# VulcanClimateModeling/fv3net

Hardware: AMD Instinct MI355X
Metric: columns/s ML-tendency inference at C384x79 (Zhao-Carr dense emulator) (higher is better)
Workload: dtype f32

## Files before the change

fv3net_amd/csrc/mlp.hip:

```cpp
#include <cmath>
#include <cstddef>
#include <cstdlib>
#include <cstring>
#include <algorithm>
#include <type_traits>
#include <cfloat>
#include <vector>

#include "common.h"

namespace fv3hip {
namespace {

#define MLP_CHUNK_BARRIER() asm volatile("s_waitcnt lgkmcnt(0)\n\ts_barrier" ::: "memory")

#define MLP_SLOT_SCHED(NT, Q)                                                          \
    __builtin_amdgcn_sched_group_barrier(0x008, 1, 0);                                 \
    __builtin_amdgcn_sched_group_barrier(0x002 | 0x400, 64, 0);                        \
    _Pragma("unroll") for (int _i = 1; _i < (NT); ++_i)                                \
    {                                                                                  \
        __builtin_amdgcn_sched_group_barrier(0x008, 1, 0);                             \
        __builtin_amdgcn_sched_group_barrier(0x004 | 0x010 | 0x080, (Q), 0);           \
    }                                                                                  \
    __builtin_amdgcn_sched_barrier(0)

typedef float f32x16 __attribute__((ext_vector_type(16)));
typedef float f32x4 __attribute__((ext_vector_type(4)));

constexpr int kMaxSources = 16;
constexpr int kMaxOutputs = 32;
constexpr int kMaxK = 2048;
constexpr int kThreads = 256;
constexpr int kTileSamples = 128;

struct KEntry {
    int src;
    int feat;
    float center;
    float scale;
    int transform;
    float eps;
    int pad0, pad1;
};

struct XAddr {
    int64_t row;
    unsigned int ss;
    unsigned int pad;
};

struct XNorm {
    float center, rscale, eps;
    int flags;
};

struct OFast {
    int64_t row;
    float scale, center;
};
struct OSlow {
    float lo, hi, mask;
    unsigned int ss;
};
struct ORes {
    int64_t src_row;
    int64_t out_row;
    unsigned int src_ss, out_ss, pad0, pad1;
};

struct OEntry {
    float scale, center, lo, hi;
    float mask;
    int out_feat;
    int res;
    int pad0;
};

struct MlpLaunch {
    unsigned int w_bytes;
    const f32x4 *w;
    const KEntry *ktab;
    const OEntry *otab;
    const float *bias;
    int n_chunks1;
    int n_hidden;
    int n_otiles;
    int n_hout_tiles;
    int smallf_off;
    int smallf_n;
    int64_t sink;
    int n_ktab;
    int n_otab;
    int n_bias;
    int out64;
    int n_log_chunks;
    int n_logfast_chunks;
    int epi_fast;
    int has_limits;
    int n_residual;
    int64_t n_samples;
    int64_t n_tiles;
    unsigned long long *stamps;
    const void *src[kMaxSources];
    int64_t src_fs[kMaxSources];
    int64_t src_ss[kMaxSources];
    void *out[kMaxOutputs];
    int64_t out_fs[kMaxOutputs];
    int64_t out_ss[kMaxOutputs];
};

__host__ __device__ constexpr int rho(int r) { return (r & 3) + 8 * (r >> 2); }

#ifndef MLP_STAMP_PHASE
#define MLP_STAMP_PHASE 0
#endif
#ifdef MLP_STAMPS
#define SLOT_STAMP(phase, s)                                          \
    if ((phase) == MLP_STAMP_PHASE) {                                 \
        const unsigned long long t_ = __builtin_readcyclecounter();   \
        if ((s) > 0) sl_acc[(s) - 1] += t_ - sl_t;                    \
        sl_t = t_;                                                    \
    }
#define CHUNK_STAMP_END(phase, KC)                                    \
    if ((phase) == MLP_STAMP_PHASE) {                                 \
        const unsigned long long t_ = __builtin_readcyclecounter();   \
        sl_acc[(KC) - 1] += t_ - sl_t;                                \
        sl_acc[16] += 1;                                              \
    }
#else
#define SLOT_STAMP(phase, s) ((void)0)
#define CHUNK_STAMP_END(phase, KC) ((void)0)
#endif
template <int HT, bool SRC64, bool XBULK, bool HOUT, bool SMALLF, bool L1SHORT>
__global__ __launch_bounds__(kThreads, 1) void mlp_fused_kernel(const MlpLaunch p)
{
    constexpr int HG = (HT + 3) / 4;
    constexpr int KC_H = 16;
    constexpr int GS = (HT == 1) ? 4 : 8;
    constexpr int NGO = GS / 4;
    constexpr int KC_O = HT * 16 / GS;
    constexpr int CH_H = KC_H * HG * 64;
    constexpr int CH_O = KC_O * NGO * 64;
    constexpr int NV_H = CH_H / kThreads;
    constexpr int NV_O = CH_O / kThreads;
    constexpr int NV_MAX = (NV_H > NV_O) ? NV_H : NV_O;
    constexpr int CH_MAX = (CH_H > CH_O) ? CH_H : CH_O;
    constexpr bool EPI_SIDE = XBULK && KC_O >= 12;

    extern __shared__ __attribute__((aligned(16))) char smem[];
    f32x4 *wbuf = reinterpret_cast<f32x4 *>(smem);
    float *xs = reinterpret_cast<float *>(wbuf + 2 * CH_MAX);
    XAddr *xa_tab = reinterpret_cast<XAddr *>(xs + (XBULK ? 2 * 32 * kTileSamples : 0));
    XNorm *xn_tab = reinterpret_cast<XNorm *>(xa_tab + p.n_ktab);
    OFast *ofast = reinterpret_cast<OFast *>(xn_tab + p.n_ktab);
    OSlow *oslow = reinterpret_cast<OSlow *>(ofast + p.n_otab);
    ORes *ores = reinterpret_cast<ORes *>(oslow + p.n_otab);
    float *biasl = reinterpret_cast<float *>(ores + (p.n_residual ? p.n_otab : 0));

    const int tid = threadIdx.x;
    const int lane = tid & 63;
    const int wave = tid >> 6;
    const int half = lane >> 5;

    {
        typedef const int64_t __attribute__((address_space(4))) *KargPtr64;
        typedef const char __attribute__((address_space(4))) *KargBytes64;
        KargPtr64 ksrc = (KargPtr64)((KargBytes64)__builtin_amdgcn_kernarg_segment_ptr() + offsetof(MlpLaunch, src));
        for (int i = tid; i < p.n_ktab; i += kThreads) {
            const KEntry e = p.ktab[i];
            const int sidx = e.src < 0 ? 0 : e.src;
            const int64_t esz = SRC64 ? 8 : 4;
            XAddr a;
            a.row = e.src < 0 ? reinterpret_cast<int64_t>(p.bias)
                              : ksrc[sidx] + (int64_t)e.feat * ksrc[kMaxSources + sidx] * esz;
            a.ss = e.src < 0 ? 0u : (unsigned int)(ksrc[2 * kMaxSources + sidx] * esz);
            a.pad = 0;
            xa_tab[i] = a;
            XNorm nrm;
            nrm.center = e.src < 0 ? 0.f : e.center;
// ... 207 lines not shown
    };
    auto bulk_finish1 = [&](int c, int i, int buf, auto with_log) {
        bulk_finish_e(xn_tab[c * 32 + fr + 8 * i], i, buf, with_log);
    };
    int xb = 0;

    int64_t tile = blockIdx.x;
    if (tile >= p.n_tiles) return;

    {
        int64_t n = tile * kTileSamples + wave * 32 + (lane & 31);
        if (XBULK) bulk_issue(0, tile * kTileSamples); else issue_x(0, n < p.n_samples ? n : p.n_samples - 1);
#pragma unroll
        for (int part = 0; part < 2; ++part) {
            issue_w(0, part);
#pragma unroll
            for (int i = 0; i < NVH; ++i) commit_w1(0, part, i);
        }
        if (XBULK) {
            if (p.n_logfast_chunks > 0) {
#pragma unroll
                for (int i = 0; i < 4; ++i) bulk_finish1(0, i, 0, std::integral_constant<int, 2>{});
            } else {
#pragma unroll
                for (int i = 0; i < 4; ++i) bulk_finish1(0, i, 0, std::integral_constant<int, 1>{});
            }
        } else {
            finish_x(0);
        }
        __syncthreads();
#pragma unroll
        for (int j = 0; j < AG; ++j) a_cur[j] = wbuf[lane + j * 64];
    }
    float b_cur = XBULK ? xs[half * kTileSamples + wave * 32 + (lane & 31)] : 0.f;

    for (; tile < p.n_tiles; tile += gridDim.x) {
        const int64_t n = tile * kTileSamples + wave * 32 + (lane & 31);
        const bool valid = n < p.n_samples;
        const int64_t nc = valid ? n : p.n_samples - 1;
        const int64_t next_tile = tile + gridDim.x;
        int64_t nn = next_tile * kTileSamples + wave * 32 + (lane & 31);
        if (nn >= p.n_samples) nn = p.n_samples - 1;
        int g = 0;

        f32x16 h[HT];
        STAMP_BEGIN();
        {
#pragma unroll
            for (int t = 0; t < HT; ++t)
#pragma unroll
                for (int r = 0; r < 16; ++r) h[t][r] = biasl[(t * 16 + r) * 2 + half];
            using T_ = std::true_type;
            using F_ = std::false_type;
            const int L = p.n_log_chunks, NC = p.n_chunks1;
            using HT_c = std::integral_constant<int, HT>;
            using HG_c = std::integral_constant<int, HG>;
            using Q5_c = std::integral_constant<int, 5>;
            auto l1_chunk = [&](int c, int cn, auto with_log) __attribute__((always_inline)) {
                const int gnext = (g + 1 < G) ? g + 1 : 0;
                const XAddr *xa_n = xa_tab + 2 * cn * KC_H + half;
                const XNorm *xn_c = xn_tab + 2 * c * KC_H + half;
                const XNorm *xn_n = xn_tab + 2 * cn * KC_H + half;
                XAddr xa_cur = xa_n[0], xa_nxt = xa_cur;
                XNorm xn_cur = xn_c[2 * (KC_H / 2)], xn_nxt = xn_cur;
#pragma unroll
                for (int s = 0; s < KC_H; ++s) {
                    run_slot(h, HT_c{}, HG_c{}, Q5_c{}, s, KC_H, xcur[s], [&](int s_) {
                        if (s_ + 1 < KC_H) {
                            xa_nxt = xa_n[2 * (s_ + 1)];
                            xn_nxt = (s_ + 1 < KC_H / 2) ? xn_c[2 * (s_ + 1 + KC_H / 2)] : xn_n[2 * (s_ + 1 - KC_H / 2)];
                        }
                        issue_x1(xa_cur, s_, nc);
                        const int el = (s_ < KC_H / 2) ? s_ + KC_H / 2 : s_ - KC_H / 2;
                        if (decltype(with_log)::value) finish_x1(xn_cur, el); else finish_x1_plain(xn_cur, el);
                        stage_step(s_, KC_H, gnext, par ^ 1);
                        xa_cur = xa_nxt;
                        xn_cur = xn_nxt;
                    });
                }
                par ^= 1;
                ++g;
            };
            auto l1_chunk_bulk = [&](int cn, int64_t n0, auto with_log, auto kc1_c) __attribute__((always_inline)) {
                constexpr int KC1 = decltype(kc1_c)::value, FIN0 = (KC1 == 16) ? 8 : 3;
                const int gnext = (g + 1 < G) ? g + 1 : 0;
                const float *xsb = xs + xb * 32 * kTileSamples + half * kTileSamples + wave * 32 + (lane & 31);
                const float *xsn = xs + (xb ^ 1) * 32 * kTileSamples + half * kTileSamples + wave * 32 + (lane & 31);
                const unsigned int nb = bulk_sample(n0);
                XAddr xa4[4];
                XNorm xn4[4];
                typedef const XAddr __attribute__((address_space(3))) *LXAddr;
                typedef const XNorm __attribute__((address_space(3))) *LXNorm;
                LXAddr xa_c = (LXAddr)(xa_tab + cn * 32 + fr);
                LXNorm xn_c = (LXNorm)(xn_tab + cn * 32 + fr);
                asm volatile("" : "+v"(xa_c), "+v"(xn_c));
                const XAddr *xa_g = (const XAddr *)xa_c;
                const XNorm *xn_g = (const XNorm *)xn_c;
#pragma unroll
                for (int s = 0; s < KC1; ++s) {
                    SLOT_STAMP((int)decltype(with_log)::value, s);
                    run_slot(h, HT_c{}, HG_c{}, Q5_c{}, s, KC1, b_cur, [&](int s_) {
                        b_cur = (s_ + 1 < KC1) ? xsb[2 * (s_ + 1) * kTileSamples] : xsn[0];
                        if (s_ == 0) {
#pragma unroll
                            for (int i = 0; i < 4; ++i) xa4[i] = xa_g[8 * i];
                        }
                        if (s_ == 1) {
#pragma unroll
                            for (int i = 0; i < 4; ++i) bulk_issue1(xa4[i], i, nb);
                        }
                        if (s_ == FIN0) {
#pragma unroll
                            for (int i = 0; i < 4; ++i) xn4[i] = xn_g[8 * i];
                        }
                        if (s_ > FIN0 && s_ <= FIN0 + 4) bulk_finish_e(xn4[s_ - FIN0 - 1], s_ - FIN0 - 1, xb ^ 1, with_log);
                        stage_step(s_, KC1, gnext, par ^ 1);
                    });
                }
                CHUNK_STAMP_END((int)decltype(with_log)::value, KC1);
                par ^= 1;
                xb ^= 1;
                ++g;
            };
            if (XBULK) {
                const int64_t n0 = tile * kTileSamples;
                using M0_ = std::integral_constant<int, 0>;
                using M1_ = std::integral_constant<int, 1>;
                using M2_ = std::integral_constant<int, 2>;
                const int NF = p.n_logfast_chunks;
                using KC16_ = std::integral_constant<int, 16>;
                const int64_t n1 = (next_tile < p.n_tiles ? next_tile : tile) * kTileSamples;
                if constexpr (L1SHORT) {
                    l1_chunk_bulk(0, n1, M0_{}, std::integral_constant<int, 8>{});
                } else {
                    int c = 0;
                    for (; c + 1 < NF; ++c) l1_chunk_bulk(c + 1, n0, M2_{}, KC16_{});
                    for (; c + 1 < L; ++c) l1_chunk_bulk(c + 1, n0, M1_{}, KC16_{});
                    for (; c < NC - 1; ++c) l1_chunk_bulk(c + 1, n0, M0_{}, KC16_{});
                    if (NF > 0) l1_chunk_bulk(0, n1, M2_{}, KC16_{});
                    else if (L > 0) l1_chunk_bulk(0, n1, M1_{}, KC16_{});
                    else l1_chunk_bulk(0, n1, M0_{}, KC16_{});
                }
            } else {
                int c = 0;
                for (; c < L && c < NC - 1; ++c) l1_chunk(c, c + 1, T_{});
                for (; c < NC - 1; ++c) l1_chunk(c, c + 1, F_{});
                if (L > 0) l1_chunk(NC - 1, NC - 1, T_{}); else l1_chunk(NC - 1, NC - 1, F_{});
            }
#pragma unroll
            for (int t = 0; t < HT; ++t)
#pragma unroll
                for (int r = 0; r < 16; ++r) h[t][r] = (h[t][r] < 0.f) ? 0.f : h[t][r];
        }
        STAMP_END(0);
        for (int l = 1; l < p.n_hidden; ++l) {
            f32x16 h2[HT];
            const float *bl = biasl + l * HT * 32;
#pragma unroll
            for (int t = 0; t < HT; ++t)
#pragma unroll
                for (int r = 0; r < 16; ++r) h2[t][r] = bl[(t * 16 + r) * 2 + half];
#pragma unroll
            for (int kt = 0; kt < HT; ++kt) {
                const int gnext = (g + 1 < G) ? g + 1 : 0;
#pragma unroll
                for (int s = 0; s < KC_H; ++s) {
                    SLOT_STAMP(10, s);
                    run_slot(h2, std::integral_constant<int, HT>{}, std::integral_constant<int, HG>{},
                             std::integral_constant<int, 2>{}, s, KC_H, h[kt][s],
                             [&](int s_) { stage_step(s_, KC_H, gnext, par ^ 1); });
                }
                CHUNK_STAMP_END(10, KC_H);
                par ^= 1;
                ++g;
            }
#pragma unroll
            for (int t = 0; t < HT; ++t)
#pragma unroll
                for (int r = 0; r < 16; ++r) h[t][r] = (h2[t][r] < 0.f) ? 0.f : h2[t][r];
        }
        STAMP_END(1);
        {
            typedef f32x4 __attribute__((address_space(1))) *GF32x4;
            typedef const f32x4 __attribute__((address_space(1))) *GCF32x4;
            typedef d64x2 __attribute__((address_space(1))) *GF64x2;
            typedef const d64x2 __attribute__((address_space(1))) *GCF64x2;
            const int64_t n0t = tile * kTileSamples + wave * 32;
            const int e_wrow = lane >> 3, e_wcol = (lane & 7) * 4;
            constexpr int NHO = HOUT ? HT : 0;
            float *scr = xs + (xb ^ 1) * 32 * kTileSamples + wave * 1024;
            auto epi_put_tile = [&](const f32x16 &y) {
#pragma unroll
                for (int r = 0; r < 16; ++r) scr[(rho(r) + 4 * half) * 32 + (lane & 31)] = y[r];
            };
            auto epi_put4 = [&](int64_t row_addr, const f32x4 v) {
                if (p.out64) {
                    const d64x2 lo = {(double)v[0], (double)v[1]}, hi = {(double)v[2], (double)v[3]};
                    *(GF64x2)(row_addr + (n0t + e_wcol) * 8) = lo;
                    *(GF64x2)(row_addr + (n0t + e_wcol) * 8 + 16) = hi;
                } else {
                    *(GF32x4)(row_addr + (n0t + e_wcol) * 4) = v;
                }
            };
            auto epi_row = [&](const OFast of, f32x4 v, int idx, auto mode_c) {
                if (decltype(mode_c)::value != 0) {
                    *(GF32x4)(of.row + (n0t + e_wcol) * 4) = v;
                    return;
                }
                if (p.has_limits) {
                    const OSlow os = oslow[idx];
#pragma unroll
                    for (int q = 0; q < 4; ++q) {
                        float x = v[q];
                        if (x < os.lo) x = os.lo;
                        if (x >= os.hi) x = os.hi;
                        v[q] = x * os.mask;
                    }
                }
                if (of.row != 0) epi_put4(of.row, v);
                if (p.n_residual) {
                    const ORes e = ores[idx];
                    if (e.src_row != 0) {
                        f32x4 before;
                        if (SRC64) {
                            const d64x2 lo = *(GCF64x2)(e.src_row + (n0t + e_wcol) * 8);
                            const d64x2 hi = *(GCF64x2)(e.src_row + (n0t + e_wcol) * 8 + 16);
                            before[0] = (float)lo[0]; before[1] = (float)lo[1];
                            before[2] = (float)hi[0]; before[3] = (float)hi[1];
                        } else {
                            before = *(GCF32x4)(e.src_row + (n0t + e_wcol) * 4);
                        }
                        epi_put4(e.out_row, before + v);
                    }
                }
            };
            auto epi_fast_now = [&](const f32x16 &y, int t) {
                if (n0t >= p.n_samples) return;
                epi_put_tile(y);
#pragma unroll
                for (int j = 0; j < 4; ++j) {
                    const int row = e_wrow + 8 * j, idx = t * 32 + row;
                    epi_row(ofast[idx], *reinterpret_cast<const f32x4 *>(scr + row * 32 + e_wcol), idx, std::integral_constant<int, 0>{});
                }
            };
            OFast e_of[2];
            f32x4 e_v[2];
            constexpr bool RES_SIDE = EPI_SIDE && !SRC64 && !HOUT && !SMALLF;
            int64_t e_src[RES_SIDE ? 4 : 1], e_out[2];
            f32x4 e_before[RES_SIDE ? 4 : 1];
            const int64_t e_loff = (n0t + e_wcol) * 4;
            auto epi_res_fetch = [&](int t, int s_, int s0) __attribute__((always_inline)) {
                if (s_ == s0) {
#pragma unroll
                    for (int j = 0; j < 4; ++j) e_src[RES_SIDE ? j : 0] = ores[t * 32 + e_wrow + 8 * j].src_row;
                }
                if (s_ == s0 + 1) {
#pragma unroll
                    for (int j = 0; j < 4; ++j) e_before[RES_SIDE ? j : 0] = *(GCF32x4)(e_src[RES_SIDE ? j : 0] + e_loff);
                }
            };
            auto epi_side = [&](const f32x16 &y, int t, int s_, auto mode_c) __attribute__((always_inline)) {
                constexpr int MODE = decltype(mode_c)::value;
                if (MODE == 0 && n0t >= p.n_samples) return;
                if (s_ == 1) epi_put_tile(y);
                if constexpr (MODE == 2 && RES_SIDE) epi_res_fetch(t, s_, 0);
                if (s_ == 9 || s_ == 10) {
#pragma unroll
                    for (int i = 0; i < 2; ++i) {
                        epi_row(e_of[i], e_v[i], t * 32 + e_wrow + 8 * (2 * (s_ - 9) + i), mode_c);
                        if constexpr (MODE == 2 && RES_SIDE)
                            *(GF32x4)(e_out[i] + e_loff) = e_before[2 * (s_ - 9) + i] + e_v[i];
                    }
                }
                if (s_ == 8 || s_ == 9) {
#pragma unroll
                    for (int i = 0; i < 2; ++i) {
                        const int row = e_wrow + 8 * (2 * (s_ - 8) + i);
                        e_of[i] = ofast[t * 32 + row];
                        e_v[i] = *reinterpret_cast<const f32x4 *>(scr + row * 32 + e_wcol);
                        if constexpr (MODE == 2 && RES_SIDE) e_out[i] = ores[t * 32 + row].out_row;
                    }
                }
            };
            auto epi_res_last = [&](const f32x16 &y, int t) {
                epi_res_fetch(t, 0, 0);
                epi_res_fetch(t, 1, 0);
                epi_put_tile(y);
                f32x4 v[4];
#pragma unroll
                for (int j = 0; j < 4; ++j) {
                    const int row = e_wrow + 8 * j;
                    v[j] = *reinterpret_cast<const f32x4 *>(scr + row * 32 + e_wcol);
                    *(GF32x4)(ofast[t * 32 + row].row + e_loff) = v[j];
                }
#pragma unroll
                for (int j = 0; j < 4; ++j)
                    *(GF32x4)(ores[t * 32 + e_wrow + 8 * j].out_row + e_loff) = e_before[RES_SIDE ? j : 0] + v[j];
            };
            auto epi_plain_last = [&](const f32x16 &y, int t) {
                epi_put_tile(y);
#pragma unroll
                for (int j = 0; j < 4; ++j) {
                    const int row = e_wrow + 8 * j;
                    *(GF32x4)(ofast[t * 32 + row].row + e_loff) = *reinterpret_cast<const f32x4 *>(scr + row * 32 + e_wcol);
                }
            };
            auto epi_general = [&](const f32x16 &y, int t) {
                typedef float __attribute__((address_space(1))) *GF32;
                typedef double __attribute__((address_space(1))) *GF64;
                const unsigned int n32 = (unsigned int)n;
#pragma unroll
                for (int gq = 0; gq < 2; ++gq) {
                    OFast of[8];
                    OSlow os[8];
                    float v[8];
#pragma unroll
                    for (int i = 0; i < 8; ++i) {
                        const int idx = t * 32 + rho(gq * 8 + i) + 4 * half;
                        of[i] = ofast[idx];
                        os[i] = oslow[idx];
                    }
#pragma unroll
                    for (int i = 0; i < 8; ++i) {
                        float x = y[gq * 8 + i];
                        if (p.has_limits) {
                            if (x < os[i].lo) x = os[i].lo;
                            if (x >= os[i].hi) x = os[i].hi;
                            x = x * os[i].mask;
                        }
                        v[i] = x;
                        if (valid && of[i].row != 0) {
                            const int64_t addr = of[i].row + (int64_t)((uint64_t)n32 * (uint64_t)os[i].ss);
                            if (p.out64)
                                *(GF64)addr = (double)x;
                            else
                                *(GF32)addr = x;
                        }
                    }
                    if (p.n_residual) {
#pragma unroll
                        for (int i = 0; i < 8; ++i) {
                            const int idx = t * 32 + rho(gq * 8 + i) + 4 * half;
                            const ORes e = ores[idx];
                            if (valid && e.src_row != 0) {
                                const float before = (float)*(GRawPtr)(e.src_row + (int64_t)((uint64_t)n32 * (uint64_t)e.src_ss));
                                const float after = before + v[i];
                                const int64_t addr = e.out_row + (int64_t)((uint64_t)n32 * (uint64_t)e.out_ss);
                                if (p.out64)
                                    *(GF64)addr = (double)after;
                                else
                                    *(GF32)addr = after;
                            }
                        }
                    }
                }
            };

            auto run_slot_out = [&](f32x16 &acc, int s, auto &&side) __attribute__((always_inline)) {
                f32x4 a_nxt[AG];
                if (s + 1 < KC_O) {
                    const f32x4 *lw = wbuf + par * CH_MAX + lane;
#pragma unroll
                    for (int j = 0; j < NGO; ++j) a_nxt[j] = lw[((s + 1) * NGO + j) * 64];
#pragma unroll
                    for (int j = NGO; j < AG; ++j) a_nxt[j] = a_cur[j];
#pragma unroll
                    for (int i = 0; i < GS; ++i)
                        acc = __builtin_amdgcn_mfma_f32_32x32x2f32(a_cur[i / 4][i % 4], h[(s * GS + i) / 16][(s * GS + i) % 16], acc, 0, 0, 0);
                    side(s);
#pragma unroll
                    for (int j = 0; j < AG; ++j) a_cur[j] = a_nxt[j];
                    MLP_SLOT_SCHED(GS, 2);
                } else {
                    acc = __builtin_amdgcn_mfma_f32_32x32x2f32(a_cur[0][0], h[(s * GS) / 16][(s * GS) % 16], acc, 0, 0, 0);
                    __builtin_amdgcn_sched_barrier(0);
                    MLP_CHUNK_BARRIER();
                    __builtin_amdgcn_sched_barrier(0);
                    const f32x4 *lwn = wbuf + (par ^ 1) * CH_MAX + lane;
#pragma unroll
                    for (int j = 0; j < AG; ++j) a_nxt[j] = lwn[j * 64];
#pragma unroll
                    for (int i = 1; i < GS; ++i)
                        acc = __builtin_amdgcn_mfma_f32_32x32x2f32(a_cur[i / 4][i % 4], h[(s * GS + i) / 16][(s * GS + i) % 16], acc, 0, 0, 0);
                    side(s);
#pragma unroll
                    for (int j = 0; j < AG; ++j) a_cur[j] = a_nxt[j];
                    MLP_SLOT_SCHED(GS - 1, 2);
                }
            };

            typedef const float __attribute__((address_space(3))) *LBias;
            auto load_bias = [&](f32x16 &y, int t) {
                const int tc = t < p.n_otiles ? t : p.n_otiles - 1;
                LBias bl = (LBias)(biasl + p.n_hidden * HT * 32 + tc * 32 + half);
                asm volatile("" : "+v"(bl));
                const float *blg = (const float *)bl;
#pragma unroll
                for (int r = 0; r < 16; ++r) y[r] = blg[r * 2];
            };
            auto out_chunk = [&](f32x16 &y, f32x16 &yo, int t, auto has_prev_c, auto mode_c) __attribute__((always_inline)) {
                const int gnext = (g + 1 == G) ? 0 : g + 1;
#pragma unroll
                for (int s = 0; s < KC_O; ++s) {
                    SLOT_STAMP(20, s);
                    run_slot_out(y, s, [&](int s_) {
                        stage_step(s_, KC_O, gnext, par ^ 1);
                        if (EPI_SIDE) {
                            if (decltype(has_prev_c)::value) epi_side(yo, NHO + t - 1, s_, mode_c);
                            if (s_ == 12) load_bias(yo, t + 1);
                        }
                    });
                }
                CHUNK_STAMP_END(20, KC_O);
                par ^= 1;
                ++g;
            };
            f32x16 yA, yB;
            const int NT = p.n_otiles;
            if constexpr (HOUT) {
                const bool prefetch_next = !XBULK && NT == 0 && next_tile < p.n_tiles;
                if (prefetch_next) issue_x(0, nn);
#pragma unroll
                for (int t = 0; t < HT; ++t) {
                    if (XBULK) epi_fast_now(h[t], t); else epi_general(h[t], t);
                }
                if (prefetch_next) finish_x(0);
            }
            if constexpr (SMALLF) {
                typedef const f32x4 __attribute__((address_space(3))) *LW4;
                LW4 wl = (LW4)(biasl + p.smallf_off + (half * 4 + (lane & 3)) * HT * 16);
                asm volatile("" : "+v"(wl));
                const f32x4 *wq = (const f32x4 *)wl;
                f32x4 acc4[4], wcur[4], wnxt[4];
#pragma unroll
                for (int i = 0; i < 4; ++i) {
                    acc4[i] = f32x4{0.f, 0.f, 0.f, 0.f};
                    wcur[i] = wq[i];
                }
#pragma unroll
                for (int t = 0; t < HT; ++t) {
#pragma unroll
                    for (int i = 0; i < 4; ++i) wnxt[i] = wq[((t + 1 < HT) ? t + 1 : t) * 4 + i];
#pragma unroll
                    for (int r = 0; r < 16; ++r)
                        acc4[r & 3] = __builtin_amdgcn_mfma_f32_4x4x1f32(wcur[r >> 2][r & 3], h[t][r], acc4[r & 3], 0, 0, 0);
#pragma unroll
                    for (int i = 0; i < 4; ++i) wcur[i] = wnxt[i];
                }
                f32x4 y4 = (acc4[0] + acc4[1]) + (acc4[2] + acc4[3]);
#pragma unroll
                for (int v = 0; v < 4; ++v) y4[v] += __shfl_xor(y4[v], 32, 64);
                if (half == 0 && n0t < p.n_samples) {
                    typedef float __attribute__((address_space(1))) *GF32;
                    const float *bo = biasl + p.n_hidden * HT * 32;
#pragma unroll
                    for (int v = 0; v < 4; ++v)
                        if (v < p.smallf_n) *(GF32)(ofast[NHO * 32 + v].row + (n0t + lane) * 4) = y4[v] + bo[2 * v];
                }
            }
            auto tile_loop = [&](auto mode_c) __attribute__((always_inline)) {
                if constexpr (EPI_SIDE) {
                    load_bias(yA, 0);
                    out_chunk(yA, yB, 0, std::false_type{}, mode_c);
                    for (int t = 1; t < NT; t += 2) {
                        out_chunk(yB, yA, t, std::true_type{}, mode_c);
                        if (t + 1 < NT) out_chunk(yA, yB, t + 1, std::true_type{}, mode_c);
                    }
                } else {
                    for (int t = 0; t < NT; ++t) {
                        load_bias(yA, t);
                        out_chunk(yA, yB, t, std::false_type{}, mode_c);
                        const bool prefetch_next = (t + 1 == NT) && next_tile < p.n_tiles;
                        if (!XBULK && prefetch_next) issue_x(0, nn);
                        if (XBULK) epi_fast_now(yA, NHO + t); else epi_general(yA, NHO + t);
                        if (!XBULK && prefetch_next) finish_x(0);
                    }
                }
            };
            bool done = false, res_last = false, plain_last = false;
            if constexpr (!SMALLF) {
            if (!HOUT || NT > 0) {
                const bool side_plain = EPI_SIDE && !p.has_limits && !p.out64 && (tile + 1) * kTileSamples <= p.n_samples;
                if (side_plain && !p.n_residual) {
                    tile_loop(std::integral_constant<int, 1>{});
// ... 413 lines not shown
#pragma unroll
    for (int ft = 0; ft < 2; ++ft)
#pragma unroll
        for (int r = 0; r < 16; ++r) acc[ft][0][r] = acc[ft][1][r] = p.b[f0 + 32 * ft + rho(r) + 4 * half];
    float a0[2][U], b0[2][U], a1[2][U], b1[2][U];
    auto load = [&](float (&a)[2][U], float (&b)[2][U], int p0) {
#pragma unroll
        for (int u = 0; u < U; ++u) {
            const int pr = (p0 + u < n_pairs) ? p0 + u : n_pairs - 1;
            a[0][u] = wl[(int64_t)2 * pr * p.fp];
            a[1][u] = wl[(int64_t)2 * pr * p.fp + 32];
            b[0][u] = xl[(int64_t)2 * pr * p.np];
            b[1][u] = xl[(int64_t)2 * pr * p.np + 32];
        }
    };
    auto mfma = [&](const float (&a)[2][U], const float (&b)[2][U]) {
#pragma unroll
        for (int u = 0; u < U; ++u)
#pragma unroll
            for (int ft = 0; ft < 2; ++ft)
#pragma unroll
                for (int st = 0; st < 2; ++st) acc[ft][st] = __builtin_amdgcn_mfma_f32_32x32x2f32(a[ft][u], b[st][u], acc[ft][st], 0, 0, 0);
    };
    load(a0, b0, 0);
    for (int p0 = 0; p0 < n_pairs; p0 += 2 * U) {
        load(a1, b1, p0 + U);
        mfma(a0, b0);
        load(a0, b0, p0 + 2 * U);
        mfma(a1, b1);
    }
#pragma unroll
    for (int ft = 0; ft < 2; ++ft)
#pragma unroll
        for (int st = 0; st < 2; ++st)
#pragma unroll
            for (int r = 0; r < 16; ++r) {
                float v = acc[ft][st][r];
                if (p.relu) v = v < 0.f ? 0.f : v;
                p.y[(int64_t)(f0 + 32 * ft + rho(r) + 4 * half) * p.np + s0 + 32 * st + col] = v;
            }
}

template <bool SRC64>
__global__ __launch_bounds__(256) void layered_scatter_kernel(const LayeredIo p)
{
    using Raw = typename std::conditional<SRC64, double, float>::type;
    const int f = blockIdx.y;
    const int64_t j = (int64_t)blockIdx.x * 256 + threadIdx.x, ns = p.n0 + j;
    const OEntry e = p.otab[f];
    if (e.out_feat < 0 || ns >= p.n_samples) return;
    float x = p.x[(int64_t)f * p.np + j];
    if (p.has_limits) {
        if (x < e.lo) x = e.lo;
        if (x >= e.hi) x = e.hi;
        x = x * e.mask;
    }
    const int slot = e.out_feat >> 20, q = e.out_feat & 0xFFFFF;
    const int64_t at = (int64_t)q * p.out_fs[slot] + ns * p.out_ss[slot];
    if (p.out64) static_cast<double *>(p.out[slot])[at] = (double)x;
    else static_cast<float *>(p.out[slot])[at] = x;
    if (e.res >= 0) {
        const int rslot = e.res >> 8, rs = e.res & 0xFF;
        const float before = (float)static_cast<const Raw *>(p.src[rs])[(int64_t)q * p.src_fs[rs] + ns * p.src_ss[rs]];
        const int64_t rat = (int64_t)q * p.out_fs[rslot] + ns * p.out_ss[rslot];
        if (p.out64) static_cast<double *>(p.out[rslot])[rat] = (double)(before + x);
        else static_cast<float *>(p.out[rslot])[rat] = before + x;
    }
}

}
}

using namespace fv3hip;

struct fv3hip_mlp {
    int device = 0;
    int HT = 0;
    int n_sources = 0, n_inputs = 0, K = 0, width = 0, n_hidden = 0, n_outputs = 0, F = 0, n_residual = 0;
    int n_chunks1 = 0, n_otiles = 0, n_hout_tiles = 0, n_ktab = 0, n_otab = 0, n_bias = 0;
    int smallf_off = 0, smallf_n = 0;
    int64_t flops = 0;
    int has_limits = 0;
    int n_log_chunks = 0, n_logfast_chunks = 0;
    unsigned int w_bytes = 0;
    void *d_sink = nullptr;
    size_t sink_bytes = 0;
    void *d_w = nullptr, *d_ktab = nullptr, *d_otab = nullptr, *d_bias = nullptr;
    void *d_w1 = nullptr, *d_wh = nullptr, *d_wo = nullptr, *d_bh = nullptr, *d_bo = nullptr;
    int Wp = 0, Fp = 0;
    int64_t small_limit = -1;
    int layered = 0, relu = 1;
    void *d_scr[2] = {nullptr, nullptr};
    size_t scr_bytes = 0;
    int n_cu = 256;
    size_t lds_bytes = 0;
    char last_variant[160] = {0};
};

namespace {

const int kHiddenTilings[] = {1, 2, 4, 8};

template <int HT, bool SRC64, bool XBULK, bool HOUT = false, bool SMALLF = false, bool L1SHORT = false>
int launch_one(const MlpLaunch &lp, int grid, size_t lds, hipStream_t st)
{
    auto kern = mlp_fused_kernel<HT, SRC64, XBULK, HOUT, SMALLF, L1SHORT>;
    FV3HIP_CHECK_HIP(hipFuncSetAttribute(reinterpret_cast<const void *>(kern),
                                         hipFuncAttributeMaxDynamicSharedMemorySize, (int)lds));
    hipLaunchKernelGGL(kern, dim3(grid), dim3(kThreads), lds, st, lp);
    return check_launch("mlp_fused_kernel");
}

template <typename T>
int upload(const std::vector<T> &v, void **dptr)
{
    *dptr = nullptr;
    if (v.empty()) return FV3HIP_OK;
    FV3HIP_CHECK_HIP(hipMalloc(dptr, v.size() * sizeof(T)));
    FV3HIP_CHECK_HIP(hipMemcpy(*dptr, v.data(), v.size() * sizeof(T), hipMemcpyHostToDevice));
    return FV3HIP_OK;
}

struct InputTable {
    std::vector<KEntry> ktab;
    std::vector<int> perm;
    int n_log_padded = 0;
    bool eps_normal = true;
};

void build_input_table(const fv3hip_mlp_desc_t *d, int K, int n_ktab, InputTable &t)
{
    t.ktab.assign(n_ktab, KEntry{-1, 0, 0.f, 1.f, 0, 0.f, 0, 0});
    t.perm.clear();
    t.perm.reserve(n_ktab);
    std::vector<KEntry> orig(K);
    int k = 0;
    for (int i = 0; i < d->n_inputs; ++i)
        for (int f = 0; f < d->in_nfeat[i]; ++f, ++k) {
            KEntry &e = orig[k];
            e = KEntry{-1, 0, 0.f, 1.f, 0, 0.f, 0, 0};
            e.src = d->in_source[i];
            e.feat = d->in_feat_start[i] + f;
            e.center = d->in_center ? d->in_center[k] : 0.f;
            e.scale = d->in_scale ? (float)(1.0 / (double)d->in_scale[k]) : 1.f;
            e.transform = d->in_transform ? d->in_transform[i] : 0;
            e.eps = d->in_eps ? d->in_eps[i] : 0.f;
        }
    for (int k2 = 0; k2 < K; ++k2)
        if (orig[k2].transform == FV3HIP_TRANSFORM_LOG) t.perm.push_back(k2);
    const int n_log = (int)t.perm.size();
    const int n_pad = (32 - n_log % 32) % 32;
    if (n_log > 0 && n_log + n_pad + (K - n_log) <= n_ktab)
        for (int i = 0; i < n_pad; ++i) t.perm.push_back(-1);
    t.n_log_padded = (int)t.perm.size();
    for (int k2 = 0; k2 < K; ++k2)
        if (orig[k2].transform != FV3HIP_TRANSFORM_LOG) t.perm.push_back(k2);
    for (size_t k2 = 0; k2 < t.perm.size(); ++k2) {
        if (t.perm[k2] >= 0) {
            t.ktab[k2] = orig[t.perm[k2]];
        } else {
            t.ktab[k2].transform = FV3HIP_TRANSFORM_LOG;
            t.ktab[k2].eps = 1.f;
        }
    }
    t.eps_normal = true;
    for (int k2 = 0; k2 < t.n_log_padded; ++k2) t.eps_normal = t.eps_normal && t.ktab[k2].eps >= FLT_MIN;
}

void build_output_table(const fv3hip_mlp_desc_t *d, int n_otab, int first_out, int n_hidden_rows, std::vector<OEntry> &otab)
{
    otab.assign(n_otab, OEntry{1.f, 0.f, -INFINITY, INFINITY, 1.f, -1, -1, 0});
    for (int q = 0; q < n_hidden_rows; ++q) otab[q].out_feat = ((d->n_outputs + d->n_residual) << 20) | q;
    int f = 0;
    for (int j = 0; j < d->n_outputs; ++j) {
        int res = -1;
        for (int r = 0; r < d->n_residual; ++r)
            if (d->res_output[r] == j) res = ((d->n_outputs + r) << 8) | d->res_source[r];
        for (int q = 0; q < d->out_nfeat[j]; ++q, ++f) {
            OEntry &e = otab[first_out + f];
            e.scale = d->out_scale ? d->out_scale[f] : 1.f;
            e.center = d->out_center ? d->out_center[f] : 0.f;
            e.lo = d->out_min ? d->out_min[f] : -INFINITY;
            e.hi = d->out_max ? d->out_max[f] : INFINITY;
            e.mask = d->out_mask ? d->out_mask[f] : 1.f;
            e.out_feat = (j << 20) | q;
            e.res = res;
        }
    }
}

}

namespace {

inline int round_up(int v, int m) { return (v + m - 1) / m * m; }

int create_layered(const fv3hip_mlp_desc_t *d, int K, fv3hip_mlp_t *out)
{
    int F = 0;
    for (int j = 0; j < d->n_outputs; ++j) {
        FV3HIP_REQUIRE(d->out_nfeat[j] >= 1 && d->out_nfeat[j] < (1 << 20), "bad out_nfeat[%d]", j);
        F += d->out_nfeat[j];
    }
    for (int r = 0; r < d->n_residual; ++r) {
        FV3HIP_REQUIRE(d->res_source[r] >= 0 && d->res_source[r] < d->n_sources, "res_source[%d] out of range", r);
        FV3HIP_REQUIRE(d->res_output[r] >= 0 && d->res_output[r] < d->n_outputs, "res_output[%d] out of range", r);
    }
    const int nh = d->n_hidden, width = nh ? d->width : K;
    FV3HIP_REQUIRE(K < 65536 && F < 65536 && width < 65536, "more than 65 535 features in a layer");
    fv3hip_mlp *m = new fv3hip_mlp();
    hipGetDevice(&m->device);
    hipDeviceProp_t prop;
    if (hipGetDeviceProperties(&prop, m->device) == hipSuccess) m->n_cu = prop.multiProcessorCount;
    m->layered = 1;
    m->relu = d->hidden_activation == FV3HIP_ACT_RELU;
    m->n_sources = d->n_sources;
    m->n_inputs = d->n_inputs;
    m->K = K;
    m->width = width;
    m->n_hidden = nh;
    m->n_outputs = d->n_outputs;
    m->F = F;
    m->n_residual = d->n_residual;
    m->has_limits = (d->out_min || d->out_max || d->out_mask) ? 1 : 0;
    m->n_ktab = round_up(K, 32);
    m->Wp = nh ? round_up(width, 64) : 0;
    m->Fp = round_up(F, 64);
    m->n_otab = m->Fp;
    m->flops = nh ? 2 * ((int64_t)K * width + (int64_t)(nh - 1) * width * width + (int64_t)width * F) : 2 * (int64_t)K * F;
    InputTable it;
    build_input_table(d, K, m->n_ktab, it);
    std::vector<OEntry> otab;
    build_output_table(d, m->n_otab, 0, 0, otab);
// ... 104 lines not shown

extern "C" int fv3hip_mlp_create(const fv3hip_mlp_desc_t *d, fv3hip_mlp_t *out)
{
    FV3HIP_REQUIRE(d && out, "null pointer");
    *out = nullptr;
    FV3HIP_REQUIRE(d->n_sources >= 1 && d->n_sources <= kMaxSources, "n_sources must be in [1, %d], got %d", kMaxSources, d->n_sources);
    FV3HIP_REQUIRE(d->n_inputs >= 1, "n_inputs must be >= 1");
    const int hout = d->hidden_output ? 1 : 0;
    FV3HIP_REQUIRE(d->n_outputs >= 1 || (d->n_outputs == 0 && hout), "n_outputs must be >= 1 (or 0 with hidden_output)");
    FV3HIP_REQUIRE(d->n_residual >= 0 && d->n_outputs + d->n_residual + hout <= kMaxOutputs,
                   "n_outputs + n_residual (+ the hidden output) must be <= %d", kMaxOutputs);
    FV3HIP_REQUIRE(d->width >= 1, "width must be >= 1");
    FV3HIP_REQUIRE(d->n_hidden >= 0, "negative n_hidden");
    FV3HIP_REQUIRE(d->hidden_activation == FV3HIP_ACT_RELU || d->hidden_activation == FV3HIP_ACT_LINEAR, "unknown activation %d", d->hidden_activation);

    int K = 0;
    for (int i = 0; i < d->n_inputs; ++i) {
        FV3HIP_REQUIRE(d->in_source[i] >= 0 && d->in_source[i] < d->n_sources, "in_source[%d] out of range", i);
        FV3HIP_REQUIRE(d->in_nfeat[i] >= 1 && d->in_feat_start[i] >= 0, "bad feature range for input %d", i);
        K += d->in_nfeat[i];
    }
    const bool layered = d->n_hidden < 1 || d->width > 256 || K > kMaxK || d->hidden_activation != FV3HIP_ACT_RELU;
    if (layered) {
        if (hout) return fail(FV3HIP_EUNSUPPORTED, "hidden-output models need 1+ ReLU hidden layers of width <= 256 and <= %d inputs", kMaxK);
        FV3HIP_REQUIRE(d->n_hidden == 0 || d->width >= 1, "width must be >= 1");
        return create_layered(d, K, out);
    }
    int F = 0;
    for (int j = 0; j < d->n_outputs; ++j) {
        FV3HIP_REQUIRE(d->out_nfeat[j] >= 1 && d->out_nfeat[j] < (1 << 20), "bad out_nfeat[%d]", j);
        F += d->out_nfeat[j];
    }
    for (int r = 0; r < d->n_residual; ++r) {
        FV3HIP_REQUIRE(d->res_source[r] >= 0 && d->res_source[r] < d->n_sources, "res_source[%d] out of range", r);
        FV3HIP_REQUIRE(d->res_output[r] >= 0 && d->res_output[r] < d->n_outputs, "res_output[%d] out of range", r);
    }

    const int width = d->width;
    const int nt_out = (F + 31) / 32;
    int HT = 0;
    for (int v : kHiddenTilings)
        if (!HT && v * 32 >= width) HT = v;
    FV3HIP_REQUIRE(HT > 0, "no kernel variant for width %d", width);

    fv3hip_mlp *m = new fv3hip_mlp();
    hipGetDevice(&m->device);
    hipDeviceProp_t prop;
    if (hipGetDeviceProperties(&prop, m->device) == hipSuccess) m->n_cu = prop.multiProcessorCount;
    m->HT = HT;
    m->n_sources = d->n_sources;
    m->n_inputs = d->n_inputs;
    m->K = K;
    m->width = width;
    m->n_hidden = d->n_hidden;
    m->n_outputs = d->n_outputs;
    m->F = F;
    m->n_residual = d->n_residual;
    m->has_limits = (d->out_min || d->out_max || d->out_mask) ? 1 : 0;
    m->n_chunks1 = ((K + 1) / 2 + 15) / 16;
    m->n_otiles = nt_out;
    m->n_ktab = 2 * 16 * m->n_chunks1;
    m->n_hout_tiles = hout ? HT : 0;
    m->n_otab = 32 * (m->n_hout_tiles + nt_out);
    m->n_bias = d->n_hidden * HT * 32 + nt_out * 32;
    if (F >= 1 && F <= 4 && !m->has_limits && d->n_residual == 0) {
        m->smallf_n = F;
        m->smallf_off = m->n_bias;
        m->n_bias += HT * 32 * 4;
    }
    m->flops = 2 * ((int64_t)K * width + (int64_t)(d->n_hidden - 1) * width * width + (int64_t)width * F);

    const int HG = (HT + 3) / 4;
    const int GS = (HT == 1) ? 4 : 8, NGO = GS / 4, KC_O = HT * 16 / GS;
    const int64_t CH_H = 16 * HG * 64, CH_O = (int64_t)KC_O * NGO * 64;
    const int n_hid_chunks = m->n_chunks1 + (d->n_hidden - 1) * HT;
    const int n_out_chunks = nt_out;

    InputTable it;
    build_input_table(d, K, m->n_ktab, it);
    std::vector<KEntry> &ktab = it.ktab;
    std::vector<int> &perm = it.perm;
    m->n_log_chunks = (it.n_log_padded + 31) / 32;
    m->n_logfast_chunks = it.eps_normal ? it.n_log_padded / 32 : 0;
    std::vector<float> w((size_t)(n_hid_chunks * CH_H + n_out_chunks * CH_O + (CH_H > CH_O ? CH_H : CH_O)) * 4, 0.f);
    auto hid_slot = [&](int g, int s, int j, int lane, int e) -> float & {
        return w[(size_t)((g * CH_H + ((int64_t)(s * HG + j) * 64 + lane)) * 4 + e)];
    };
    {
        const float *W = d->hidden_kernels[0];
        for (int g = 0; g < m->n_chunks1; ++g)
            for (int s = 0; s < 16; ++s)
                for (int j = 0; j < HG; ++j)
                    for (int lane = 0; lane < 64; ++lane)
                        for (int e = 0; e < 4; ++e) {
                            const int k = 2 * (g * 16 + s) + (lane >> 5);
                            const int f = 32 * (4 * j + e) + (lane & 31);
                            if (k < (int)perm.size() && perm[k] >= 0 && f < width)
                                hid_slot(g, s, j, lane, e) = W[(size_t)perm[k] * width + f] * ktab[k].scale;
                        }
    }
    for (int l = 1; l < d->n_hidden; ++l) {
        const float *W = d->hidden_kernels[l];
        for (int kt = 0; kt < HT; ++kt) {
            const int g = m->n_chunks1 + (l - 1) * HT + kt;
            for (int s = 0; s < 16; ++s)
                for (int j = 0; j < HG; ++j)
                    for (int lane = 0; lane < 64; ++lane)
                        for (int e = 0; e < 4; ++e) {
                            const int k = 32 * kt + rho(s) + 4 * (lane >> 5);
                            const int f = 32 * (4 * j + e) + (lane & 31);
                            if (k < width && f < width) hid_slot(g, s, j, lane, e) = W[(size_t)k * width + f];
                        }
        }
    }
    {
        const float *W = d->out_kernel;
        const size_t base = (size_t)n_hid_chunks * CH_H * 4;
        for (int t = 0; t < nt_out; ++t)
            for (int s = 0; s < KC_O; ++s)
                for (int j = 0; j < NGO; ++j)
                    for (int lane = 0; lane < 64; ++lane)
                        for (int e = 0; e < 4; ++e) {
                            const int mm = GS * s + 4 * j + e;
                            const int k = 32 * (mm / 16) + rho(mm % 16) + 4 * (lane >> 5);
                            const int f = 32 * t + (lane & 31);
                            if (k < width && f < F)
                                w[base + (size_t)((t * CH_O + ((int64_t)(s * NGO + j) * 64 + lane)) * 4 + e)] =
                                    W[(size_t)k * F + f] * (d->out_scale ? d->out_scale[f] : 1.f);
                        }
    }
    std::vector<OEntry> otab;
    build_output_table(d, m->n_otab, 32 * m->n_hout_tiles, hout ? width : 0, otab);
    std::vector<float> bias(m->n_bias, 0.f);
    for (int l = 0; l < d->n_hidden; ++l)
        for (int t = 0; t < HT; ++t)
            for (int r = 0; r < 16; ++r)
                for (int hf = 0; hf < 2; ++hf) {
                    const int f = 32 * t + rho(r) + 4 * hf;
                    if (f < width) bias[(size_t)l * HT * 32 + (t * 16 + r) * 2 + hf] = d->hidden_biases[l][f];
                }
    for (int t = 0; t < nt_out; ++t)
        for (int r = 0; r < 16; ++r)
            for (int hf = 0; hf < 2; ++hf) {
                const int f = 32 * t + rho(r) + 4 * hf;
                if (f < F)
                    bias[(size_t)d->n_hidden * HT * 32 + (size_t)t * 32 + r * 2 + hf] =
                        (float)((double)d->out_bias[f] * (d->out_scale ? d->out_scale[f] : 1.f) + (d->out_center ? d->out_center[f] : 0.f));
            }

    if (m->smallf_n)
        for (int hf = 0; hf < 2; ++hf)
            for (int f = 0; f < F; ++f)
                for (int t = 0; t < HT; ++t)
                    for (int r = 0; r < 16; ++r) {
                        const int k = 32 * t + rho(r) + 4 * hf;
                        if (k < width)
                            bias[(size_t)m->smallf_off + (size_t)(((hf * 4 + f) * HT + t) * 16 + r)] =
                                d->out_kernel[(size_t)k * F + f] * (d->out_scale ? d->out_scale[f] : 1.f);
                    }

    const int Wp = HT * 32, Fp = (nt_out > 0 ? nt_out : 1) * 32;
    m->Wp = Wp;
    m->Fp = Fp;
    std::vector<float> w1((size_t)m->n_ktab * Wp, 0.f), wh((size_t)(d->n_hidden > 1 ? d->n_hidden - 1 : 1) * Wp * Wp, 0.f),
        wo((size_t)Wp * Fp, 0.f), bh((size_t)d->n_hidden * Wp, 0.f), bo((size_t)Fp, 0.f);
    for (size_t k = 0; k < perm.size(); ++k)
// ... 113 lines not shown
        lp.out_ss[j] = out_sample_stride[j];
    }
    if (m->layered) return predict_layered(m, lp, src64, out_dtype, n_samples, as_stream(stream));
    {
        static const int64_t small_max = [] {
            const char *e = getenv("FV3HIP_MLP_SMALL_MAX_SAMPLES");
            return e ? (int64_t)atoll(e) : (int64_t)-1;
        }();
        const int64_t limit = m->small_limit >= 0 ? m->small_limit : small_max >= 0 ? small_max : (int64_t)32 * m->n_cu;
        const size_t lds_small = (size_t)(2 * kSmallChunk * 32 + 2 * m->Wp * 32) * sizeof(float) + (size_t)m->n_ktab * 32 +
                                 (size_t)3 * (kMaxOutputs + kMaxSources) * sizeof(int64_t);
        if (n_samples <= limit && m->n_otiles + m->n_hout_tiles > 0 && lds_small <= 160 * 1024) {
            SmallLaunch sp;
            memset(&sp, 0, sizeof(sp));
            sp.w1 = static_cast<const float *>(m->d_w1);
            sp.wh = static_cast<const float *>(m->d_wh);
            sp.wo = static_cast<const float *>(m->d_wo);
            sp.bh = static_cast<const float *>(m->d_bh);
            sp.bo = static_cast<const float *>(m->d_bo);
            sp.ktab = static_cast<const KEntry *>(m->d_ktab);
            sp.otab = static_cast<const OEntry *>(m->d_otab);
            sp.n_ktab = m->n_ktab;
            sp.Wp = m->Wp;
            sp.HT = m->HT;
            sp.n_hidden = m->n_hidden;
            sp.Fp = m->Fp;
            sp.n_otiles = m->n_otiles;
            sp.n_hout_tiles = m->n_hout_tiles;
            sp.out64 = (out_dtype == FV3HIP_F64);
            sp.has_limits = m->has_limits;
            sp.n_samples = n_samples;
#ifdef SMALL_STAMPS
            sp.stamps = g_small_stamps;
#endif
            memcpy(sp.src, lp.src, sizeof(sp.src));
            memcpy(sp.src_fs, lp.src_fs, sizeof(sp.src_fs));
            memcpy(sp.src_ss, lp.src_ss, sizeof(sp.src_ss));
            memcpy(sp.out, lp.out, sizeof(sp.out));
            memcpy(sp.out_fs, lp.out_fs, sizeof(sp.out_fs));
            memcpy(sp.out_ss, lp.out_ss, sizeof(sp.out_ss));
            const int grid_s = (int)ceil_div(n_samples, (int64_t)32);
            hipStream_t st_s = as_stream(stream);
            snprintf(m->last_variant, sizeof(m->last_variant), "mlp_small_kernel<%s> (32-sample workgroups, features split over %d waves)",
                     src64 ? "true" : "false", kSmallWaves);
            if (src64) {
                auto kern = mlp_small_kernel<true>;
                FV3HIP_CHECK_HIP(hipFuncSetAttribute(reinterpret_cast<const void *>(kern), hipFuncAttributeMaxDynamicSharedMemorySize, (int)lds_small));
                hipLaunchKernelGGL(kern, dim3(grid_s), dim3(kSmallWaves * 64), lds_small, st_s, sp);
            } else {
                auto kern = mlp_small_kernel<false>;
                FV3HIP_CHECK_HIP(hipFuncSetAttribute(reinterpret_cast<const void *>(kern), hipFuncAttributeMaxDynamicSharedMemorySize, (int)lds_small));
                hipLaunchKernelGGL(kern, dim3(grid_s), dim3(kSmallWaves * 64), lds_small, st_s, sp);
            }
            return check_launch("mlp_small_kernel");
        }
    }
    lp.w = static_cast<const f32x4 *>(m->d_w);
    lp.w_bytes = m->w_bytes;
    lp.ktab = static_cast<const KEntry *>(m->d_ktab);
    lp.otab = static_cast<const OEntry *>(m->d_otab);
    lp.bias = static_cast<const float *>(m->d_bias);
    lp.n_chunks1 = m->n_chunks1;
    lp.n_hidden = m->n_hidden;
    lp.n_otiles = m->n_otiles;
    lp.n_hout_tiles = m->n_hout_tiles;
    lp.n_ktab = m->n_ktab;
    lp.n_otab = m->n_otab;
    lp.n_bias = m->n_bias;
    lp.out64 = (out_dtype == FV3HIP_F64);
    lp.has_limits = m->has_limits;
    {
        const int oal = (out_dtype == FV3HIP_F64) ? 2 : 4, sal = src64 ? 2 : 4;
        bool fast = (n_samples % 32 == 0);
        for (int j = 0; j < n_slots && fast; ++j)
            fast = out_sample_stride[j] == 1 && (reinterpret_cast<uintptr_t>(outputs[j]) % 16 == 0) &&
                   (out_feat_stride[j] % oal == 0);
        for (int i = 0; i < m->n_sources && fast; ++i)
            fast = src_sample_stride[i] == 1 && (reinterpret_cast<uintptr_t>(sources[i]) % 16 == 0) &&
                   (src_feat_stride[i] % sal == 0);
        lp.epi_fast = fast ? 1 : 0;
    }
    lp.n_log_chunks = m->n_log_chunks;
    lp.n_logfast_chunks = m->n_logfast_chunks;
    lp.n_residual = m->n_residual;
    lp.n_samples = n_samples;
    lp.n_tiles = ceil_div(n_samples, kTileSamples);
#ifdef MLP_STAMPS
    lp.stamps = g_mlp_stamps;
#endif
    const int grid = (int)(lp.n_tiles < m->n_cu ? lp.n_tiles : m->n_cu);
    bool xbulk = lp.epi_fast != 0;
    hipStream_t st = as_stream(stream);
    constexpr size_t kLdsMax = 160 * 1024, kXsBytes = 2 * 32 * kTileSamples * sizeof(float);
    if (m->lds_bytes + kXsBytes > kLdsMax) xbulk = false;
    const size_t lds = m->lds_bytes + (xbulk ? kXsBytes : 0);
    lp.sink = 0;
    if (xbulk) {
        const size_t need = (size_t)n_samples * 8;
        if (m->sink_bytes < need) {
            if (m->d_sink) FV3HIP_CHECK_HIP(hipFree(m->d_sink));
            m->d_sink = nullptr;
            m->sink_bytes = 0;
            FV3HIP_CHECK_HIP(hipMalloc(&m->d_sink, need));
            m->sink_bytes = need;
        }
        lp.sink = reinterpret_cast<int64_t>(m->d_sink);
    }
    if (m->n_hout_tiles && src64)
        return fail(FV3HIP_EUNSUPPORTED, "hidden-output models take float32 sources only");
    const bool smallf = m->smallf_n && xbulk && !src64 && out_dtype == FV3HIP_F32;
    if (smallf) {
        lp.n_otiles = 0;
        lp.smallf_off = m->smallf_off;
        lp.smallf_n = m->smallf_n;
    }
    const bool l1short = smallf && !m->n_hout_tiles && m->K <= 16 && m->n_log_chunks == 0;
    {
        const bool hout_v = m->n_hout_tiles != 0;
        const bool src64_v = src64 && !smallf && !hout_v;
        const bool side = xbulk && !smallf && m->HT == 8 && !m->has_limits && out_dtype == FV3HIP_F32 && n_samples >= kTileSamples;
        const char *epi = smallf ? "small-output" : (side && !m->n_residual) ? "plain"
                          : (side && !src64_v && !hout_v) ? "residual" : "general";
        snprintf(m->last_variant, sizeof(m->last_variant), "mlp_fused_kernel<%d,%s,%s,%s,%s,%s> epilogue=%s", m->HT,
                 src64_v ? "true" : "false", xbulk ? "true" : "false", hout_v ? "true" : "false",
                 smallf ? "true" : "false", l1short ? "true" : "false", epi);
    }
#define VARIANT_(H)                                                                                \
    if (m->HT == H && l1short) return launch_one<H, false, true, false, true, true>(lp, grid, lds, st); \
    if (m->HT == H && smallf)                                                                      \
        return m->n_hout_tiles ? launch_one<H, false, true, true, true>(lp, grid, lds, st)         \
                               : launch_one<H, false, true, false, true>(lp, grid, lds, st);       \
    if (m->HT == H && m->n_hout_tiles)                                                             \
        return xbulk ? launch_one<H, false, true, true>(lp, grid, lds, st) : launch_one<H, false, false, true>(lp, grid, lds, st); \
    if (m->HT == H) {                                                                              \
        if (xbulk) return src64 ? launch_one<H, true, true>(lp, grid, lds, st) : launch_one<H, false, true>(lp, grid, lds, st); \
        return src64 ? launch_one<H, true, false>(lp, grid, lds, st) : launch_one<H, false, false>(lp, grid, lds, st);          \
    }
#ifndef MLP_FAST_BUILD
    VARIANT_(1)
    VARIANT_(2)
    VARIANT_(4)
#endif
    VARIANT_(8)
#undef VARIANT_
    return fail(FV3HIP_EUNSUPPORTED, "no compiled kernel variant for HT=%d", m->HT);
}
```

Baseline: 195.1 million.

## Use half-length first-layer chunk after partial log chunk and prebias epilogue LDS pointers

When the log-transformed inputs leave a partially filled trailing 32-wide chunk (1 to 16 real features), the first layer now runs the chunk after the log chunks as an 8-slot short chunk instead of a full 16-slot one, with the log finishes batched into one slot. This cuts MFMA slots for zero-padded K columns. Separately, the residual epilogue uses base LDS pointers computed once per output chunk instead of recomputing table indices every slot. The risk is correctness if the short chunk does not line up with the padded weight layout, plus scheduling changes from batching the finishes.

```diff
diff --git a/fv3net_amd/csrc/mlp.hip b/fv3net_amd/csrc/mlp.hip
--- a/fv3net_amd/csrc/mlp.hip
+++ b/fv3net_amd/csrc/mlp.hip
@@ -95,6 +95,7 @@
     int out64;
     int n_log_chunks;
     int n_logfast_chunks;
+    int l1_short_log;
     int epi_fast;
     int has_limits;
     int n_residual;
@@ -468,7 +469,10 @@
                 ++g;
             };
             auto l1_chunk_bulk = [&](int cn, int64_t n0, auto with_log, auto kc1_c) __attribute__((always_inline)) {
-                constexpr int KC1 = decltype(kc1_c)::value, FIN0 = (KC1 == 16) ? 8 : 3;
+                constexpr int KC1 = decltype(kc1_c)::value;
+                constexpr bool SHORT_LOG = KC1 == 8 && !L1SHORT;
+                constexpr int FIN0 = (KC1 == 16) ? 8 : SHORT_LOG ? 5 : 3;
+                constexpr int SPH = SHORT_LOG ? 3 : (int)decltype(with_log)::value;
                 const int gnext = (g + 1 < G) ? g + 1 : 0;
                 const float *xsb = xs + xb * 32 * kTileSamples + half * kTileSamples + wave * 32 + (lane & 31);
                 const float *xsn = xs + (xb ^ 1) * 32 * kTileSamples + half * kTileSamples + wave * 32 + (lane & 31);
@@ -484,7 +488,7 @@
                 const XNorm *xn_g = (const XNorm *)xn_c;
 #pragma unroll
                 for (int s = 0; s < KC1; ++s) {
-                    SLOT_STAMP((int)decltype(with_log)::value, s);
+                    SLOT_STAMP(SPH, s);
                     run_slot(h, HT_c{}, HG_c{}, Q5_c{}, s, KC1, b_cur, [&](int s_) {
                         b_cur = (s_ + 1 < KC1) ? xsb[2 * (s_ + 1) * kTileSamples] : xsn[0];
                         if (s_ == 0) {
@@ -499,11 +503,18 @@
 #pragma unroll
                             for (int i = 0; i < 4; ++i) xn4[i] = xn_g[8 * i];
                         }
-                        if (s_ > FIN0 && s_ <= FIN0 + 4) bulk_finish_e(xn4[s_ - FIN0 - 1], s_ - FIN0 - 1, xb ^ 1, with_log);
+                        if constexpr (SHORT_LOG) {
+                            if (s_ == FIN0 + 1) {
+#pragma unroll
+                                for (int i = 0; i < 4; ++i) bulk_finish_e(xn4[i], i, xb ^ 1, with_log);
+                            }
+                        } else {
+                            if (s_ > FIN0 && s_ <= FIN0 + 4) bulk_finish_e(xn4[s_ - FIN0 - 1], s_ - FIN0 - 1, xb ^ 1, with_log);
+                        }
                         stage_step(s_, KC1, gnext, par ^ 1);
                     });
                 }
-                CHUNK_STAMP_END((int)decltype(with_log)::value, KC1);
+                CHUNK_STAMP_END(SPH, KC1);
                 par ^= 1;
                 xb ^= 1;
                 ++g;
@@ -522,6 +533,10 @@
                     int c = 0;
                     for (; c + 1 < NF; ++c) l1_chunk_bulk(c + 1, n0, M2_{}, KC16_{});
                     for (; c + 1 < L; ++c) l1_chunk_bulk(c + 1, n0, M1_{}, KC16_{});
+                    if (p.l1_short_log) {
+                        l1_chunk_bulk(c + 1, n0, M0_{}, std::integral_constant<int, 8>{});
+                        ++c;
+                    }
                     for (; c < NC - 1; ++c) l1_chunk_bulk(c + 1, n0, M0_{}, KC16_{});
                     if (NF > 0) l1_chunk_bulk(0, n1, M2_{}, KC16_{});
                     else if (L > 0) l1_chunk_bulk(0, n1, M1_{}, KC16_{});
@@ -635,21 +650,23 @@
             int64_t e_src[RES_SIDE ? 4 : 1], e_out[2];
             f32x4 e_before[RES_SIDE ? 4 : 1];
             const int64_t e_loff = (n0t + e_wcol) * 4;
-            auto epi_res_fetch = [&](int t, int s_, int s0) __attribute__((always_inline)) {
+            auto epi_res_fetch = [&](const ORes *ob, int s_, int s0) __attribute__((always_inline)) {
                 if (s_ == s0) {
 #pragma unroll
-                    for (int j = 0; j < 4; ++j) e_src[RES_SIDE ? j : 0] = ores[t * 32 + e_wrow + 8 * j].src_row;
+                    for (int j = 0; j < 4; ++j) e_src[RES_SIDE ? j : 0] = ob[8 * j].src_row;
                 }
                 if (s_ == s0 + 1) {
 #pragma unroll
                     for (int j = 0; j < 4; ++j) e_before[RES_SIDE ? j : 0] = *(GCF32x4)(e_src[RES_SIDE ? j : 0] + e_loff);
                 }
             };
+            const OFast *e_ofb = ofast;
+            const ORes *e_orb = ores;
             auto epi_side = [&](const f32x16 &y, int t, int s_, auto mode_c) __attribute__((always_inline)) {
                 constexpr int MODE = decltype(mode_c)::value;
                 if (MODE == 0 && n0t >= p.n_samples) return;
                 if (s_ == 1) epi_put_tile(y);
-                if constexpr (MODE == 2 && RES_SIDE) epi_res_fetch(t, s_, 0);
+                if constexpr (MODE == 2 && RES_SIDE) epi_res_fetch(e_orb, s_, 0);
                 if (s_ == 9 || s_ == 10) {
 #pragma unroll
                     for (int i = 0; i < 2; ++i) {
@@ -662,15 +679,19 @@
 #pragma unroll
                     for (int i = 0; i < 2; ++i) {
                         const int row = e_wrow + 8 * (2 * (s_ - 8) + i);
-                        e_of[i] = ofast[t * 32 + row];
+                        if constexpr (MODE == 2 && RES_SIDE) {
+                            e_of[i] = e_ofb[8 * (2 * (s_ - 8) + i)];
+                            e_out[i] = e_orb[8 * (2 * (s_ - 8) + i)].out_row;
+                        } else {
+                            e_of[i] = ofast[t * 32 + row];
+                        }
                         e_v[i] = *reinterpret_cast<const f32x4 *>(scr + row * 32 + e_wcol);
-                        if constexpr (MODE == 2 && RES_SIDE) e_out[i] = ores[t * 32 + row].out_row;
                     }
                 }
             };
             auto epi_res_last = [&](const f32x16 &y, int t) {
-                epi_res_fetch(t, 0, 0);
-                epi_res_fetch(t, 1, 0);
+                epi_res_fetch(ores + t * 32 + e_wrow, 0, 0);
+                epi_res_fetch(ores + t * 32 + e_wrow, 1, 0);
                 epi_put_tile(y);
                 f32x4 v[4];
 #pragma unroll
@@ -786,6 +807,15 @@
             };
             auto out_chunk = [&](f32x16 &y, f32x16 &yo, int t, auto has_prev_c, auto mode_c) __attribute__((always_inline)) {
                 const int gnext = (g + 1 == G) ? 0 : g + 1;
+                if constexpr (decltype(mode_c)::value == 2 && RES_SIDE && decltype(has_prev_c)::value) {
+                    typedef const OFast __attribute__((address_space(3))) *LOFast;
+                    typedef const ORes __attribute__((address_space(3))) *LORes;
+                    LOFast ofb = (LOFast)(ofast + (NHO + t - 1) * 32 + e_wrow);
+                    LORes orb = (LORes)(ores + (NHO + t - 1) * 32 + e_wrow);
+                    asm volatile("" : "+v"(ofb), "+v"(orb));
+                    e_ofb = (const OFast *)ofb;
+                    e_orb = (const ORes *)orb;
+                }
 #pragma unroll
                 for (int s = 0; s < KC_O; ++s) {
                     SLOT_STAMP(20, s);
@@ -1365,6 +1395,7 @@
     int64_t flops = 0;
     int has_limits = 0;
     int n_log_chunks = 0, n_logfast_chunks = 0;
+    int l1_short_log = 0;
     unsigned int w_bytes = 0;
     void *d_sink = nullptr;
     size_t sink_bytes = 0;
@@ -1407,6 +1438,7 @@
 struct InputTable {
     std::vector<KEntry> ktab;
     std::vector<int> perm;
+    int n_log = 0;
     int n_log_padded = 0;
     bool eps_normal = true;
 };
@@ -1432,6 +1464,7 @@
     for (int k2 = 0; k2 < K; ++k2)
         if (orig[k2].transform == FV3HIP_TRANSFORM_LOG) t.perm.push_back(k2);
     const int n_log = (int)t.perm.size();
+    t.n_log = n_log;
     const int n_pad = (32 - n_log % 32) % 32;
     if (n_log > 0 && n_log + n_pad + (K - n_log) <= n_ktab)
         for (int i = 0; i < n_pad; ++i) t.perm.push_back(-1);
@@ -1702,6 +1735,7 @@
     std::vector<int> &perm = it.perm;
     m->n_log_chunks = (it.n_log_padded + 31) / 32;
     m->n_logfast_chunks = it.eps_normal ? it.n_log_padded / 32 : 0;
+    m->l1_short_log = (it.n_log_padded % 32 == 0 && it.n_log % 32 >= 1 && it.n_log % 32 <= 16 && m->n_log_chunks < m->n_chunks1) ? 1 : 0;
     std::vector<float> w((size_t)(n_hid_chunks * CH_H + n_out_chunks * CH_O + (CH_H > CH_O ? CH_H : CH_O)) * 4, 0.f);
     auto hid_slot = [&](int g, int s, int j, int lane, int e) -> float & {
         return w[(size_t)((g * CH_H + ((int64_t)(s * HG + j) * 64 + lane)) * 4 + e)];
@@ -1981,6 +2015,7 @@
     }
     lp.n_log_chunks = m->n_log_chunks;
     lp.n_logfast_chunks = m->n_logfast_chunks;
+    lp.l1_short_log = m->l1_short_log;
     lp.n_residual = m->n_residual;
     lp.n_samples = n_samples;
     lp.n_tiles = ceil_div(n_samples, kTileSamples);
```

Measured after the change: 197.8 million (median of 6 runs). 1.01x the previous value.
